# mariohsouto/ProxSDP.jl

Measured on AMD Instinct MI355X. Metric: PDHG iterations/sec at target rank ~ sqrt(n), Max-Cut SDP n=4000 (tol 1e-4 options), higher is better.
Workload: dtype f64

## Files before the change

include/proxsdp_hip.h:

```cpp
#ifndef PROXSDP_HIP_H
#define PROXSDP_HIP_H

#include <stdint.h>

#ifdef __cplusplus
extern "C" {
#endif

#define PROXSDP_HIP_ABI_VERSION 10

#define PROXSDP_E_INVALID  (-1)
#define PROXSDP_E_HIP      (-2)
#define PROXSDP_E_NOMEM    (-3)
#define PROXSDP_E_UNSUPP   (-4)
#define PROXSDP_E_INTERNAL (-5)
#define PROXSDP_E_COMM_ABORTED (-6)

#define PROXSDP_STATUS_NOT_CALLED       0
#define PROXSDP_STATUS_OPTIMAL          1
#define PROXSDP_STATUS_TIME_LIMIT       2
#define PROXSDP_STATUS_ITERATION_LIMIT  3
#define PROXSDP_STATUS_INFEAS_OR_UNBND  4
#define PROXSDP_STATUS_DUAL_INFEASIBLE  5
#define PROXSDP_STATUS_INFEASIBLE       6
// ... 166 lines not shown
    double  host_eig_overlap_time;
    int64_t sign_short_pass;
    int64_t sign_short_fail;
    int64_t full_eigs_lanczos_certified;
    int64_t full_eigs_lanczos_cert_failed;
    int64_t cert_matvecs;
    int64_t dense_truncated_projections;
    int64_t wide_krylov_projections;
    int64_t reserved_s[4];
    int64_t dense_setup_passes;
    int64_t dense_sigma_steps;
} proxsdp_stats;
#define PROXSDP_STATS_SHARDED_GENERAL_ITERATIONS 0
#define PROXSDP_STATS_DEVICE_EIG_MERGES 1
#define PROXSDP_STATS_DEVICE_EIG_MERGE_FALLBACKS 2

typedef struct proxsdp_result {
    int32_t status;
    int32_t certificate_found;
    int32_t primal_feasible_user_tol;
    int32_t dual_feasible_user_tol;
    int32_t result_count;
    int32_t final_rank;
    int64_t iter;
    double  primal_residual;
    double  dual_residual;
    double  objval, dual_objval, gap, time;
    double  dual_feasibility;
    double* primal;
    double* dual_cone;
// ... 260 lines not shown
```

proxsdp.jl_amd/binding.py:

```python
import ctypes as C
import os
import pathlib
import re

import numpy as np
import scipy.sparse as sp

_HERE = pathlib.Path(__file__).resolve().parent
LIB_PATH = _HERE / "libproxsdp_hip.so"
HEADER_PATH = _HERE.parent / "include" / "proxsdp_hip.h"

TRACE_COLS = 14
TRACE_NAMES = ("iter", "prim_obj", "dual_obj", "gap", "feas", "prim_res", "dual_res",
               "primal_step", "beta", "theta", "target_rank", "trials", "elapsed", "matvecs")


class LibraryNotBuilt(RuntimeError):
    pass


class ProxSDPHipError(RuntimeError):
    def __init__(self, code, msg):
        super().__init__(f"libproxsdp_hip error {code}: {msg}")
        self.code = code
# ... 105 lines not shown
                ("dense_truncated_projections", i64), ("wide_krylov_projections", i64), ("reserved_s", i64 * 4),
                ("dense_setup_passes", i64), ("dense_sigma_steps", i64)]


class Result(C.Structure):
    _fields_ = [("status", i32), ("certificate_found", i32), ("primal_feasible_user_tol", i32),
                ("dual_feasible_user_tol", i32), ("result_count", i32), ("final_rank", i32),
                ("iter", i64), ("primal_residual", f64), ("dual_residual", f64),
                ("objval", f64), ("dual_objval", f64), ("gap", f64), ("time", f64),
                ("dual_feasibility", f64),
                ("primal", pf64), ("dual_cone", pf64), ("dual_eq", pf64), ("dual_in", pf64),
                ("slack_eq", pf64), ("slack_in", pf64), ("trace", pf64), ("trace_rows", i64),
                ("status_string", C.c_char * 256), ("stats", Stats)]


STATS_RESERVED_SLOTS = {"sharded_general_iterations": 0, "device_eig_merges": 1, "device_eig_merge_fallbacks": 2}

STATE_NHIST = 7
STATE_HIST_NAMES = ("dual_gap", "prim_obj", "dual_obj", "feasibility", "primal_residual", "dual_residual", "comb_residual")
STATE_SCAL_NAMES = ("primal_step", "primal_step_old", "dual_step", "beta", "theta", "adapt_level",
                    "equa_feasibility", "ineq_feasibility", "dual_feasibility")


class State(C.Structure):
    _fields_ = [("struct_size", i64), ("iteration", i64), ("n", i64), ("Q", i64), ("n_psd", i64), ("hist_len", i64),
                ("x", pf64), ("y", pf64), ("Mty", pf64), ("Mx", pf64),
                ("target_rank", pi64), ("current_rank", pi64), ("min_eig", pf64), ("hist", pf64),
                ("scal", f64 * 16), ("ints", i64 * 8)]


class ShardIO(C.Structure):
# ... 1081 lines not shown
```

proxsdp.jl_amd/csrc/kernels.hip.hpp:

```cpp
#pragma once
#include <hip/hip_runtime.h>
#include <cstdint>

namespace proxsdp {
namespace dev {

constexpr int WAVE = 64;
constexpr int TILE = 64;
constexpr int TPB = 256;
constexpr int NWAVE = TPB / WAVE;
constexpr int CPW = TILE / NWAVE;
constexpr double INV_SQRT2 = 0.70710678118654752440;
constexpr double SQRT2 = 1.41421356237309504880;

#ifdef PX_TIMELINE
constexpr int TL_WG = 160, TL_SLOTS = 8, TL_K = 260;
__device__ unsigned long long g_tl[2][TL_K][TL_WG][TL_SLOTS];
#define PX_TL(kind, k, slot)                                                                                   \
    do {                                                                                                       \
        if (threadIdx.x == 0 && (int)blockIdx.x < ::proxsdp::dev::TL_WG && (k) >= 0 && (k) < ::proxsdp::dev::TL_K) { \
            asm volatile("" ::: "memory");                                                                     \
            ::proxsdp::dev::g_tl[kind][k][blockIdx.x][slot] = wall_clock64();                                    \
            asm volatile("" ::: "memory");                                                                     \
        }                                                                                                      \
// ... 289 lines not shown
    if (wv == 0) wbuf[i] = ((s_acc[0][lane] + s_acc[1][lane]) + (s_acc[2][lane] + s_acc[3][lane])) * INV_SQRT2;
}

__device__ __forceinline__ double fold16_all(double (&t)[16], int lane) {
    fold_stage<8>(t, lane);
    fold_stage<4>(t, lane);
    fold_stage<2>(t, lane);
    fold_stage<1>(t, lane);
    return add_xor32(add_xor16(t[0]));
}
struct FopArgs {
    const double* Vp;
    const double* lam;
    int rp;
    const double* tpart;
    const double* ebuf;
    const double* apart;
};
template <int NCH, int NCHP>
__device__ __forceinline__ void
lz_orth_body(const double* __restrict__ Ppart, int nt, int npad, const double* __restrict__ V, int ldv, int k,
             double* __restrict__ wbuf, const double* __restrict__ hred, double* __restrict__ hpart_out, int pld,
             double* __restrict__ hsum_out, const LanczosCtl* __restrict__ ctl,
             const double* __restrict__ alphas, const double* __restrict__ betas,
             const double* __restrict__ Apart, int napart, int first, const double* __restrict__ arrow, int keep,
             const FopArgs& fo) {
    PX_TL(1, k, 0);
    const int stop = ctl->stop;
    constexpr int NC = 16 * NCH;
    constexpr int NCP = 16 * (NCHP > 0 ? NCHP : 1);
    __shared__ double s_t[NWAVE * 4 * 4 * NCP];
    __shared__ double s_u[4 * NCP];
    __shared__ double s_h[4 * NC];
    __shared__ double s_q[4 * NC];
    __shared__ double s_acc[NWAVE][LZ_ROWS];
    __shared__ double s_red[NWAVE];
    const int lane = threadIdx.x & 63;
    const int wv = __builtin_amdgcn_readfirstlane((int)(threadIdx.x >> 6));
    const int i = blockIdx.x * LZ_ROWS + lane;
    double pv[16];
    double av[8];
    constexpr int NLP = (NCHP > 0 ? NCHP : 1);
    double vrp[NCP], tp[16][NLP], eb = 0.0, ap = 0.0;
    if constexpr (NCHP == 0) {
#pragma unroll
        for (int u = 0; u < 16; ++u) pv[u] = (wv + u * NWAVE < nt) ? Ppart[(long long)(wv + u * NWAVE) * npad + i] : 0.0;
#pragma unroll
        for (int u = 0; u < 8; ++u) av[u] = (u * TPB < napart) ? Apart[min((int)threadIdx.x + u * TPB, napart - 1)] : 0.0;
    } else {
        const int gl0 = min(lane, pld - 1);
#pragma unroll
        for (int c = 0; c < NCP; ++c) {
            const int cc = min(wv + 4 * c, max(fo.rp - 1, 0));
            vrp[c] = fo.Vp[(long long)cc * ldv + i];
        }
#pragma unroll
        for (int u = 0; u < 16; ++u) {
            const long long rec = (long long)min(wv + NWAVE * u, pld - 1) * RLD;
#pragma unroll
            for (int ch = 0; ch < NLP; ++ch)
                tp[u][ch] = ((ch == 0 || 64 * ch < fo.rp) && (wv + NWAVE * u < nt || pld > WAVE)) ? fo.tpart[rec + 64 * ch + lane] : 0.0;
        }
        eb = fo.ebuf[i];
        ap = fo.apart[gl0];
    }
    double vr[NC];
#pragma unroll
    for (int c0 = 0; c0 < NC; c0 += 4) {
        if (wv + 4 * c0 <= k) {
#pragma unroll
            for (int c = c0; c < c0 + 4; ++c) vr[c] = V[(long long)min(wv + 4 * c, k) * ldv + i];
        } else {
#pragma unroll
            for (int c = c0; c < c0 + 4; ++c) vr[c] = 0.0;
        }
    }
// ... 16 lines not shown
    const double binv = first ? 1.0 : 1.0 / be_km;
    if constexpr (NCHP == 0) {
#pragma unroll
        for (int u = 0; u < 16; ++u) if (wv + u * NWAVE >= nt) pv[u] = 0.0;
        double acc = (((pv[0] + pv[1]) + (pv[2] + pv[3])) + ((pv[4] + pv[5]) + (pv[6] + pv[7]))) +
                     (((pv[8] + pv[9]) + (pv[10] + pv[11])) + ((pv[12] + pv[13]) + (pv[14] + pv[15])));
        for (int s = wv + 16 * NWAVE; s < nt; s += NWAVE) acc += Ppart[(long long)s * npad + i];
        s_acc[wv][lane] = acc;
#pragma unroll
        for (int u = 0; u < 8; ++u) if ((int)threadIdx.x + u * TPB >= napart) av[u] = 0.0;
        double a = ((av[0] + av[1]) + (av[2] + av[3])) + ((av[4] + av[5]) + (av[6] + av[7]));
        for (int t = threadIdx.x + 8 * TPB; t < napart; t += TPB) a += Apart[t];
        a = wave_sum(a);
        if (lane == 0) s_red[wv] = a;
    } else {
#pragma unroll
        for (int ch = 0; ch < NLP; ++ch) {
            double pr[16], q4[4];
#pragma unroll
            for (int u = 0; u < 16; ++u) {
                pr[u] = tp[u][ch];
                if (64 * ch < fo.rp)
                    for (int g = wv + NWAVE * u + WAVE; g < pld; g += WAVE) pr[u] += fo.tpart[(long long)g * RLD + 64 * ch + lane];
            }
            tree_in_wave(pr, q4);
#pragma unroll
            for (int a = 0; a < 4; ++a) s_t[(wv * 4 + a) * (64 * NLP) + 64 * ch + lane] = q4[a];
        }
        if (lane >= pld) ap = 0.0;
        else for (int g = lane + WAVE; g < pld; g += WAVE) ap += fo.apart[g];
        ap = wave_sum(ap);
        if (lane == 0) s_red[wv] = (wv == 0) ? ap : 0.0;
    }
    if (!first && (int)threadIdx.x < 4 * NC) s_h[threadIdx.x] = ((int)threadIdx.x < k) ? hred_j : 0.0;
    __syncthreads();
    PX_TL(1, k, 3);
    double alpha, wi;
    if constexpr (NCHP == 0) {
        alpha = ((s_red[0] + s_red[1]) + (s_red[2] + s_red[3])) * INV_SQRT2 * binv * binv;
        wi = ((s_acc[0][lane] + s_acc[1][lane]) + (s_acc[2][lane] + s_acc[3][lane])) * (INV_SQRT2 * binv);
    } else {
        auto tsum = [&](int c) { return tree_across(s_t, 64 * NLP, c); };
        double tl = 0.0;
        if (lane < fo.rp) { const double t0 = tsum(lane); tl = lam_l0 * t0 * t0; }
        if constexpr (NCHP > 1) if (lane + WAVE < fo.rp) { const double t1 = tsum(lane + WAVE); tl += lam_l1 * t1 * t1; }
        tl = wave_sum(tl);
        alpha = (tl + s_red[0]) * binv * binv;
        wi = eb * binv;
        if (j < 4 * NCP) s_u[j] = (j < fo.rp) ? lam_j * tsum(j) : 0.0;
    }
    double ck = alpha;
    if (first) {
        if (j < keep) s_q[j] = f_j;
    } else {
        ck -= s_h[k - 1];
        double fh = 0.0;
        if (keep > 0 && k > keep) {
            if (lane < keep) fh = f_l0 * s_h[lane];
            if (lane + WAVE < keep) fh += f_l1 * s_h[lane + WAVE];
            for (int jj = lane + 2 * WAVE; jj < keep; jj += WAVE) fh += arrow[jj] * s_h[jj];
            fh = wave_sum(fh);
        }
        if (j < k) {
            const double hj = s_h[j];
// ... 42 lines not shown
        const double r = wave_sum(wp * wp);
        if (lane == 0) hpart_out[(long long)pld * KLD + blockIdx.x] = r;
    }
    if (blockIdx.x == 0 && threadIdx.x == 0) hsum_out[k] = ck;
#pragma unroll
    for (int ch = 0; ch < NCH; ++ch) {
        double t[16];
#pragma unroll
        for (int c = 0; c < 16; ++c) t[c] = (wv + 4 * (16 * ch + c) <= k) ? vr[16 * ch + c] * wp : 0.0;
        const double hs = fold16_all(t, lane);
        const int jc = wv + 4 * (16 * ch + lane);
        if (lane < 16 && jc <= k) hpart_out[(long long)blockIdx.x * KLD + jc] = hs;
    }
    PX_TL(1, k, 6);
}
template <int NCH, int NCHP>
__global__ void __launch_bounds__(TPB)
k_lz_orth(const double* __restrict__ Ppart, int nt, int npad, const double* __restrict__ V, int ldv, int k,
          double* __restrict__ wbuf, const double* __restrict__ hred, double* __restrict__ hpart_out, int pld,
          double* __restrict__ hsum_out, const LanczosCtl* __restrict__ ctl,
          const double* __restrict__ alphas, const double* __restrict__ betas,
          const double* __restrict__ Apart, int napart, int first, const double* __restrict__ arrow, int keep,
          FopArgs fo) {
    lz_orth_body<NCH, NCHP>(Ppart, nt, npad, V, ldv, k, wbuf, hred, hpart_out, pld, hsum_out, ctl, alphas, betas, Apart,
                            napart, first, arrow, keep, fo);
}

template <int NCH>
__device__ __forceinline__ void lz_finish_body(const double* __restrict__ wbuf, double* __restrict__ V, int ldv, int k,
                                               const double* __restrict__ hpart_in, int pld,
                                               const double* __restrict__ h1, double* __restrict__ alphas,
                                               double* __restrict__ betas, LanczosCtl* __restrict__ ctl,
                                               double tol, int use_carry, int g,
                                               double* __restrict__ s_h, double* __restrict__ s_d,
                                               double* __restrict__ s_beta, double* __restrict__ hred,
                                               int nprod ) {
    constexpr int NC = 16 * NCH;
    __shared__ double s_p[NWAVE * 4 * 64 * NCH];
    const int lane = threadIdx.x & 63;
    const int wv = __builtin_amdgcn_readfirstlane((int)(threadIdx.x >> 6));
// ... 204 lines not shown
    const LzBlk& b = B.b[blockIdx.z];
    if (b.mode == 0) return;
    FopArgs fo{};
    lz_orth_body<1, 0>(b.Ppart, B.nt, B.npad, b.V, B.npad, b.k, b.wbuf, b.hred, (b.k & 1) ? b.hpart2 : b.hpart1, B.pld,
                       b.hsum, b.ctl, b.alphas, b.betas, b.Apart, B.napart, b.k == b.keep ? 1 : 0, b.arrow, b.keep, fo);
}

struct EllOverflow {
    const int* wr_ptr;
    const int* wr_row;
    const int* wr_lo;
    const int* wr_hi;
    const int* ov_col;
    const int* ov_sidx;
};
template <int NCHP>
__device__ __forceinline__ void fop_body(const double* __restrict__ v, const double* __restrict__ Vp, int ldv, int rp,
                                         const int* __restrict__ ell_col, const int* __restrict__ ell_sidx, int ell_w,
                                         int npad, const double* __restrict__ esv, double* __restrict__ tpart, int pld,
                                         double* __restrict__ ebuf, double* __restrict__ apart, int g,
                                         double* __restrict__ s_e , const LanczosCtl* __restrict__ ctl,
                                         const EllOverflow& ov, int tlk = -1 ) {
    constexpr int NCP = 16 * NCHP;
    const int lane = threadIdx.x & 63;
    const int wv = __builtin_amdgcn_readfirstlane((int)(threadIdx.x >> 6));
    const int i = g * LZ_ROWS + lane;
    PX_TL(0, tlk, 0);
    const int stop = (ctl != nullptr) ? ctl->stop : 0;
    const double vi = v[i];
    double vrp[NCP];
#pragma unroll
    for (int c = 0; c < NCP; ++c) vrp[c] = Vp[(long long)min(wv + 4 * c, max(rp - 1, 0)) * ldv + i];
    int col0[4], sx0[4];
#pragma unroll
    for (int u = 0; u < 4; ++u) {
        const int k = min(wv + u * NWAVE, ell_w - 1);
        col0[u] = ell_col[(long long)k * npad + i];
        sx0[u] = (wv + u * NWAVE < ell_w) ? ell_sidx[(long long)k * npad + i] : -1;
    }
    if (stop) return;
    PX_TL(0, tlk, 1);
    double e = 0.0;
    for (int k0 = wv; k0 < ell_w; k0 += 4 * NWAVE) {
        int col[4], sx[4];
#pragma unroll
        for (int u = 0; u < 4; ++u) {
            if (k0 == wv) { col[u] = col0[u]; sx[u] = sx0[u]; continue; }
// ... 19 lines not shown
                const int rloc = ov.wr_row[q], grow = g * LZ_ROWS + rloc;
                double a = 0.0;
                for (int k = ov.wr_lo[q] + (int)threadIdx.x; k < ov.wr_hi[q]; k += TPB) {
                    const int col = ov.ov_col[k];
                    const double evk = esv[ov.ov_sidx[k]];
                    a += ((col == grow) ? evk : evk * INV_SQRT2) * v[col];
                }
                a = wave_sum(a);
                if (lane == 0) s_w[wv] = a;
                __syncthreads();
                if (threadIdx.x == 0) s_e[rloc] += (s_w[0] + s_w[1]) + (s_w[2] + s_w[3]);
                __syncthreads();
            }
        }
    }
#pragma unroll
    for (int ch = 0; ch < NCHP; ++ch) {
        double t[16];
#pragma unroll
        for (int c = 0; c < 16; ++c) t[c] = vrp[16 * ch + c] * vi;
        const double ts = fold16_all(t, lane);
        const int cc = wv + 4 * (16 * ch + lane);
        if (lane < 16 && cc < rp) tpart[(long long)g * RLD + cc] = ts;
    }
    __syncthreads();
    PX_TL(0, tlk, 3);
    if (wv == 0) {
        const double ei = (s_e[lane] + s_e[LZ_ROWS + lane]) + (s_e[2 * LZ_ROWS + lane] + s_e[3 * LZ_ROWS + lane]);
        ebuf[i] = ei;
        const double a = wave_sum(vi * ei);
        if (lane == 0) apart[g] = a;
    }
    PX_TL(0, tlk, 4);
}
template <int NCHP>
__global__ void __launch_bounds__(TPB)
k_fop(const double* __restrict__ v, const double* __restrict__ Vp, int ldv, int rp,
      const int* __restrict__ ell_col, const int* __restrict__ ell_sidx, int ell_w, int npad,
      const double* __restrict__ esv, double* __restrict__ tpart, int pld, double* __restrict__ ebuf,
      double* __restrict__ apart, const LanczosCtl* __restrict__ ctl, EllOverflow ov) {
    __shared__ double s_e[NWAVE * LZ_ROWS];
    fop_body<NCHP>(v, Vp, ldv, rp, ell_col, ell_sidx, ell_w, npad, esv, tpart, pld, ebuf, apart, blockIdx.x, s_e, ctl, ov);
}
template <int NCHP, int NCH>
__global__ void __launch_bounds__(TPB)
k_fop_finish(const double* __restrict__ wbuf, double* __restrict__ V, int ldv, int k,
             const double* __restrict__ hpart_in, int pld, const double* __restrict__ h1,
             double* __restrict__ alphas, double* __restrict__ betas, LanczosCtl* __restrict__ ctl, double tol,
             int use_carry, int nt, const double* __restrict__ Vp, int rp,
             const int* __restrict__ ell_col, const int* __restrict__ ell_sidx, int ell_w, int npad,
             const double* __restrict__ esv, double* __restrict__ tpart, double* __restrict__ ebuf,
             double* __restrict__ apart, double* __restrict__ hred, EllOverflow ov) {
    __shared__ double s_a[2 * NWAVE * TILE];
    __shared__ double s_b[NWAVE * LZ_ROWS];
    __shared__ double s_beta;
    if ((int)blockIdx.x < nt) {
        lz_finish_body<NCH>(wbuf, V, ldv, k, hpart_in, pld, h1, alphas, betas, ctl, tol, use_carry, blockIdx.x,
                            s_a, s_b, &s_beta, hred, nt);
    } else {
        fop_body<NCHP>(wbuf, Vp, ldv, rp, ell_col, ell_sidx, ell_w, npad, esv, tpart, pld, ebuf, apart,
                       (int)blockIdx.x - nt, s_b, ctl, ov, k + 1);
    }
}

__global__ void __launch_bounds__(TPB)
k_lz_rotate(const double* __restrict__ V, int ldv, int n, int K, const double* __restrict__ U, int ldu,
            int ncols, double* __restrict__ out, int ldo, int copy_src, int copy_dst) {
    extern __shared__ double s_mem[];
    double* s_U = s_mem;
    double* s_V = s_mem + (size_t)K * ncols;
    const int lane = threadIdx.x & 63, wv = threadIdx.x >> 6;
    const int i = blockIdx.x * LZ_ROWS + lane;
    for (int t = threadIdx.x; t < K * ncols; t += TPB) {
        const int j = t % K, c = t / K;
        s_U[t] = U[(long long)c * ldu + j];
    }
// ... 1285 lines not shown
```

proxsdp.jl_amd/csrc/lanczos.hip.hpp:

```cpp
#pragma once
#include "solver.hip.hpp"

namespace proxsdp {

struct LzRecord {
    const double* al; const double* be;
    dev::LanczosCtl ctl;
    LzRecord(const double* rec, int ld) : al(rec), be(rec + ld) { std::memcpy(&ctl, rec + 2 * ld, sizeof(ctl)); }
};

template <typename K, typename... Args>
static inline void launch_prof(EigEvents* prof, K kern, dim3 grid, hipStream_t stream, Args... args) {
    if (!prof) { hipLaunchKernelGGL(kern, grid, dim3(dev::TPB), 0, stream, args...); return; }
    const auto e = prof->acquire();
    hipExtLaunchKernelGGL(kern, grid, dim3(dev::TPB), 0, stream, e.first, e.second, 0, args...);
}
inline EigEvents* Solver::profiled_launch(EigWork& W, int phase) const {
    if (!(opt.profile_symv_every > 0 && (W.lst.symv_launches % opt.profile_symv_every) == phase)) return nullptr;
    return phase == 0 ? &W.ev : &W.evo;
}

inline void Solver::launch_symv(EigWork& W, const double* xp, const double* v, bool use_ctl, dev::LanczosCtl* ctl) {
    EigEvents* const prof = profiled_launch(W, 0);
    if (W.use_fop) {
        auto kern = (W.F_r <= 64) ? dev::k_fop<1> : dev::k_fop<2>;
        launch_prof(prof, kern, dim3(W.nt), stream,
                    v, W.prev_factors().V, W.npad, W.F_r,
                    (const int*)W.ell_col.p, (const int*)W.ell_sidx.p, W.ell_w, W.npad, W.esv, W.tpart.p, W.pld,
                    W.ebuf.p, W.apartf.p, (const dev::LanczosCtl*)(use_ctl ? W.ctl_p : nullptr), W.ov);
    } else {
        launch_prof(prof, dev::k_symv_packed, dim3(W.napart), stream,
                    xp, W.n, W.nt, W.npad, v, W.Ppart.p, (const dev::LanczosCtl*)(use_ctl ? (ctl ? ctl : W.ctl_p) : nullptr), W.Apart.p);
    }
    count_matvecs(W, 1);
}

inline double* lz_hpart(EigWork& W, int k) { return (k & 1) ? W.hpart2.p : W.hpart1.p; }

inline void Solver::launch_symv_finish(EigWork& W, const double* xp, int kclose, double tol, bool use_carry) {
    EigEvents* const prof = profiled_launch(W, 0);
    with_nch(kclose + 1, [&](auto nch) {
        constexpr int NCH = decltype(nch)::value;
        if (W.use_fop) {
            auto kern = (W.F_r <= 64) ? dev::k_fop_finish<1, NCH> : dev::k_fop_finish<2, NCH>;
            launch_prof(prof, kern, dim3(2 * W.nt), stream,
                        (const double*)W.w.p, W.V.p, W.npad, kclose, (const double*)lz_hpart(W, kclose), W.pld,
                        (const double*)W.hsum1.p, W.alphas_p, W.betas_p, W.ctl_p, tol, use_carry ? 1 : 0, W.nt,
                        W.prev_factors().V, W.F_r,
                        (const int*)W.ell_col.p, (const int*)W.ell_sidx.p, W.ell_w, W.npad, W.esv, W.tpart.p, W.ebuf.p,
                        W.apartf.p, W.hred.p, W.ov);
        } else {
            launch_prof(prof, dev::k_symv_finish<NCH>, dim3(W.nt + W.napart), stream,
                        xp, W.n, W.nt, W.npad, W.Ppart.p, (const double*)W.w.p, W.V.p, W.npad, kclose,
                        (const double*)lz_hpart(W, kclose), W.pld, (const double*)W.hsum1.p, W.alphas_p, W.betas_p, W.ctl_p,
                        tol, use_carry ? 1 : 0, W.Apart.p, W.hred.p);
        }
    });
    count_matvecs(W, 1);
}

inline void Solver::lz_launch_finish(EigWork& W, int k, double tol, bool use_carry) {
    with_nch(k + 1, [&](auto nch) {
        hipLaunchKernelGGL(dev::k_lz_finish<decltype(nch)::value>, dim3(W.nt), dim3(dev::TPB), 0, stream,
                           (const double*)W.w.p, W.n, W.V.p, W.npad, k, (const double*)lz_hpart(W, k), W.pld,
                           (const double*)W.hsum1.p, W.alphas_p, W.betas_p, W.ctl_p, tol, use_carry ? 1 : 0, W.hred.p);
    });
}

inline void Solver::lz_launch_begin(EigWork& W, const double* start, dev::LanczosCtl* ctl) {
    hipLaunchKernelGGL(dev::k_lz_begin, dim3(ceil_div(W.npad, dev::TPB)), dim3(dev::TPB), 0, stream,
                       W.V.p, start, W.npad, ctl);
}

inline void Solver::lz_launch_orth(EigWork& W, int k, int first, int keep, EigEvents* prof) {
    dev::FopArgs fo{};
    if (W.use_fop) {
        const EigWork::Factors F = W.prev_factors();
        fo.Vp = F.V; fo.lam = F.lam; fo.rp = F.r;
        fo.tpart = W.tpart.p; fo.ebuf = W.ebuf.p; fo.apart = W.apartf.p;
    }
    auto launch_orth = [&](auto kern) {
        launch_prof(prof, kern, dim3(W.nt), stream,
                    (const double*)W.Ppart.p, W.nt, W.npad, (const double*)W.V.p, W.npad, k, W.w.p,
                    (const double*)W.hred.p, lz_hpart(W, k), W.pld, W.hsum1.p,
                    (const dev::LanczosCtl*)W.ctl_p, (const double*)W.alphas_p, (const double*)W.betas_p,
                    (const double*)W.Apart.p, W.napart, first, (const double*)W.arrow_p, keep, fo);
    };
    with_nch(k + 1, [&](auto nch) {
        constexpr int NCH = decltype(nch)::value;
        if (!W.use_fop) launch_orth(dev::k_lz_orth<NCH, 0>);
        else if (W.F_r <= 64) launch_orth(dev::k_lz_orth<NCH, 1>);
        else launch_orth(dev::k_lz_orth<NCH, 2>);
    });
}

inline void Solver::lz_first_matvec(EigWork& W, const double* xp, int k, bool& presymv, dev::LanczosCtl* ctl) {
    if (!presymv) launch_symv(W, xp, W.V.p + (size_t)k * W.npad, true, ctl);
    else count_matvecs(W, 1);
    presymv = false;
}

inline void Solver::lz_launch_step(EigWork& W, const double* xp, int k, int kfirst, double step_tol, bool& presymv) {
    if (k == kfirst) lz_first_matvec(W, xp, k, presymv, W.ctl_p);
    else launch_symv_finish(W, xp, k - 1, step_tol, k - 1 > kfirst);
    lz_launch_orth(W, k, k == kfirst ? 1 : 0, kfirst, profiled_launch(W, 1));
}

// ... 187 lines not shown
    return true;
}

inline void Solver::lz_plan(EigWork& W, LzRun& R, bool single_block) {
    LzPlan& p = R.plan;
    const int krylovdim = R.krylovdim;
    const bool wide = krylovdim > dev::LZ_KMAX;
    const int merge_from = opt.host_eig_merge == 0 ? (1 << 30) : (opt.host_eig_merge == 1 ? 24 : 64);
    const bool split_wanted = single_block && !R.arpack && krylovdim >= merge_from;
    const bool blk1 = single_block && !wide && block1_plan(W, krylovdim, split_wanted);
    p.engine = wide ? LzEngine::wide : blk1 ? LzEngine::block1 : LzEngine::step;
    p.rec = W.record(wide);
    p.split = p.engine == LzEngine::step && split_wanted;
    p.dev_wanted = p.split && (opt.device_eig_merge == 1 || (opt.device_eig_merge < 0 && krylovdim >= 64));
    p.dev_merge = p.dev_wanted && rot_sink == nullptr && StreamRef::tl == nullptr && DeviceMerge::eligible(krylovdim);
}

inline void Solver::lz_prepare_arrow(LzRun& R) {
    R.m_arrow = R.kfirst;
    if (R.m_arrow <= 0) return;
    const int n1 = R.m_arrow + 1, ld = R.ld;
    R.Qa.assign((size_t)n1 * n1, 0.0); R.da.assign(n1, 0.0); R.ea.assign(n1, 0.0);
    for (int j = 0; j < R.m_arrow; ++j) {
        R.Qa[(size_t)j * n1 + j] = R.T[(size_t)j * ld + j];
        R.Qa[(size_t)j * n1 + R.m_arrow] = R.Qa[(size_t)R.m_arrow * n1 + j] = R.T[(size_t)j * ld + R.m_arrow];
    }
    householder_tridiag(n1, R.Qa.data(), R.da.data(), R.ea.data());
}

inline bool Solver::lz_split_first(EigWork& W, LzRun& R) {
// ... 562 lines not shown
```

proxsdp.jl_amd/csrc/pdhg_loop.hip.hpp:

```cpp
#pragma once
#include "solver.hip.hpp"

namespace proxsdp {

constexpr int PSTRIDE = 2048;
constexpr int NQ = 16;

inline void Solver::spmv(const double* x, double* y) {
    spmv_sparse(x, y);
    if (P.dense()) dense_mv(x, y, true);
}
inline void Solver::spmv_sparse(const double* x, double* y) {
    if (P.Q == 0) return;
    if (csr_wave)
        hipLaunchKernelGGL(dev::k_spmv_csr_wave, dim3(ceil_div(P.Q, dev::NWAVE)), dim3(dev::TPB), 0, stream,
                           csr_ptr.p, csr_col.p, csr_val.p, x, y, (int)P.Q, LONG_ROW);
    else
        hipLaunchKernelGGL(dev::k_spmv_csr_thread, dim3(ceil_div(P.Q, dev::TPB)), dim3(dev::TPB), 0, stream,
                           csr_ptr.p, csr_col.p, csr_val.p, x, y, (int)P.Q, LONG_ROW);
    if (n_seg > 0) {
        hipLaunchKernelGGL(dev::k_spmv_csr_seg, dim3(n_seg), dim3(dev::TPB), 0, stream,
                           seg_lo_d.p, seg_hi_d.p, csr_col.p, csr_val.p, x, segpart_d.p);
        hipLaunchKernelGGL(dev::k_spmv_seg_fin, dim3(ceil_div(n_long, dev::TPB)), dim3(dev::TPB), 0, stream,
                           long_row_d.p, long_ptr_d.p, n_long, segpart_d.p, y);
// ... 820 lines not shown
                        whi.push_back((int)ocol.size());
                    }
                    wptr[g + 1] = (int)wrow.size();
                }
                W.wr_ptr.alloc(wptr.size()); W.wr_row.alloc(wrow.size()); W.wr_lo.alloc(wlo.size()); W.wr_hi.alloc(whi.size());
                W.ov_col.alloc(ocol.size()); W.ov_sidx.alloc(osx.size());
                W.wr_ptr.upload(wptr.data(), wptr.size(), stream); W.wr_row.upload(wrow.data(), wrow.size(), stream);
                W.wr_lo.upload(wlo.data(), wlo.size(), stream); W.wr_hi.upload(whi.data(), whi.size(), stream);
                W.ov_col.upload(ocol.data(), ocol.size(), stream); W.ov_sidx.upload(osx.data(), osx.size(), stream);
                W.ov = dev::EllOverflow{W.wr_ptr.p, W.wr_row.p, W.wr_lo.p, W.wr_hi.p, W.ov_col.p, W.ov_sidx.p};
                PX_HIP(hipStreamSynchronize(stream));
            }
            W.F.alloc((size_t)W.npad * W.cap); W.F.zero(stream);
            W.Flam.alloc(std::max(W.n, dev::MAXK)); W.Flam.zero(stream);
            W.tpart.alloc((size_t)dev::MAXK * W.pld); W.tpart.zero(stream);
            W.ebuf.alloc(W.npad); W.ebuf.zero(stream);
            W.apartf.alloc(W.pld); W.apartf.zero(stream);
            W.warm_part.alloc(ceil_div(W.npad, dev::TPB)); W.warm_part.zero(stream);
            PX_HIP(hipStreamSynchronize(stream));
            W.fop_ok = true;
        }
    }
    PX_HIP(hipStreamSynchronize(stream));
    use_support = true;
}

inline void Solver::upload_sparse_operator() {
    std::vector<int> rp(P.Q + 1), cp(P.n + 1);
    for (int64_t i = 0; i <= P.Q; ++i) rp[i] = (int)P.rowptr[i];
    for (int64_t i = 0; i <= P.n; ++i) cp[i] = (int)P.colptr[i];
// ... 689 lines not shown
```

proxsdp.jl_amd/csrc/solver.hip.hpp:

```cpp
#pragma once
#include <hip/hip_runtime.h>
#include <hip/hip_ext.h>
#include <array>
#include <memory>
#include <mutex>
#include <condition_variable>
#include <functional>
#include <exception>
#include <rocblas/rocblas.h>
#include <rocsolver/rocsolver.h>

#include <algorithm>
#include <chrono>
#include <cmath>
#include <cstdio>
#include <cstdlib>
#include <cstring>
#include <stdexcept>
#include <string>
#include <thread>
#include <tuple>
#include <type_traits>
#include <utility>
#include <vector>
// ... 172 lines not shown

struct StreamRef {
    Stream main;
    static inline thread_local hipStream_t tl = nullptr;
    operator hipStream_t() const { return tl ? tl : main.h; }
};

struct LzRecBuf { double* dev = nullptr; double* host = nullptr; size_t doubles = 0; int ld = 0; dev::LanczosCtl* ctl = nullptr; };
enum class LzEngine { step, block1, wide };
struct LzPlan {
    LzEngine engine = LzEngine::step;
    LzRecBuf rec;
    bool split = false;
    bool dev_wanted = false;
    bool dev_merge = false;
};
struct LzRun {
    LzPlan plan;
    int nev = 0, krylovdim = 0, ld = 0;
    bool arpack = false, positive_part = false;
    double tol = 0.0, step_tol = 0.0;
    long long maxiter = 0;
    std::vector<double> T, Tw, D, U, f, al, be, Qa, da, ea;
    int howmany = 0, numiter = 1, converged = 0, K = 0, kfirst = 0, pos_count = -1, m_arrow = 0;
    bool pos_fail = false, presymv = false;
    double betaK = 0.0;
    int k1 = 0;
    bool split_cycle = false, split_ready = false;
    bool merge_active = false;
    bool dev_staged = false;
// ... 23 lines not shown
    dev::LanczosCtl* ctlw_p = nullptr;
    static constexpr size_t RECW_DOUBLES = 2 * dev::LZW_MAXK + sizeof(dev::LanczosCtl) / sizeof(double);
    LzRecBuf record(bool wide_one) const {
        if (wide_one) return {recw.p, recw_pinned.p, RECW_DOUBLES, dev::LZW_MAXK, ctlw_p};
        return {rec.p, rec_host, REC_DOUBLES, dev::MAXK, ctl_p};
    }
    DevBuf<double> A, D, E;
    DevBuf<rocblas_int> info;
    std::vector<double> resid_host;
    PinnedBuf Ustage[2];
    int ustage_next = 0;
    int rot_form = 0, rot_launches = 0;
    std::vector<double> vals;
    int count = 0, converged_eigs = 0, numiter = 0, prev_numiter = 1;
    bool converged = false;
    DevBuf<double> F, Flam, tpart, ebuf, apartf;
    DevBuf<int> ell_col, ell_sidx;
    DevBuf<int> wr_ptr, wr_row, wr_lo, wr_hi, ov_col, ov_sidx;
    dev::EllOverflow ov{};
    int ell_w = 0, F_first = 0, F_r = 0;
    bool fop_ok = false;
    bool have_factors = false;
    bool use_fop = false;
    struct XPrev {
        bool sparse = true;
        int last_npos = -1;
    } xprev;
    struct Factors { const double* V; const double* lam; int r; };
    Factors prev_factors() const { return {F.p + (size_t)F_first * npad, Flam.p, F_r}; }
    void forget_factors() { have_factors = false; xprev.sparse = false; use_fop = false; }
    bool ritz_ok = false;
// ... 129 lines not shown
    struct BatchCtx {
        DevBuf<double> U;
        PinnedBuf U_host, rec_host;
        std::unique_ptr<SpinPool> pool;
        Event ev;
    };
    std::vector<std::unique_ptr<BatchCtx>> batch_ctx;
    std::mutex batch_stats_mu;
    std::unique_ptr<SpinPool> merge_pool;
    ParFor merge_par;
    int merge_helpers() const { return opt.host_merge_threads < 0 ? 3 : std::min(15, (int)opt.host_merge_threads); }
    static constexpr size_t LZB_USTRIDE = 64 * 64 + 2 * dev::MAXK;
    int block1_lds_cap = 0;
    DevBuf<long long> b1_dbg;
    bool sg48_ok = false;
    EigEvents* profiled_launch(EigWork& W, int phase) const;
    void launch_symv(EigWork& W, const double* xp, const double* v, bool use_ctl, dev::LanczosCtl* ctl = nullptr);
    void launch_symv_finish(EigWork& W, const double* xp, int kclose, double tol, bool use_carry);
    void lz_launch_finish(EigWork& W, int k, double tol, bool use_carry);
    void lz_launch_begin(EigWork& W, const double* start, dev::LanczosCtl* ctl);
    void lz_launch_orth(EigWork& W, int k, int first, int keep, EigEvents* prof);
    void lz_first_matvec(EigWork& W, const double* xp, int k, bool& presymv, dev::LanczosCtl* ctl);
    void lz_launch_step(EigWork& W, const double* xp, int k, int kfirst, double step_tol, bool& presymv);
    void lzw_step(EigWork& W, LzRun& R, const double* xp, int k);
    bool block1_plan(const EigWork& W, int krylovdim, bool split_wanted) const;
    void launch_block1(EigWork& W, const double* xp, int kfirst, int krylovdim, double tol);
    void lz_read_record(const LzRecBuf& rec, double* dst, hipStream_t s);
    void rotate(EigWork& W, int K, const std::vector<double>& U, int ldu, int ncols, double* out, int copy_src, int copy_dst,
                const double* extra, int nextra);
    void rotate_launch(EigWork& W, int K, const double* Ud, int ncols, double* out, int copy_src, int copy_dst);
// ... 332 lines not shown
    sg48_ok = true;
    for (const void* f : {reinterpret_cast<const void*>(dev::k_sym_gemm48<dev::SG_PLAIN, 4>), reinterpret_cast<const void*>(dev::k_sym_gemm48<dev::SG_POLY, 4>)})
        sg48_ok = sg48_ok && hipFuncSetAttribute(f, hipFuncAttributeMaxDynamicSharedMemorySize, (int)dev::sg48_lds_bytes(4)) == hipSuccess;
    if (!sg48_ok) (void)hipGetLastError();
    small_sign_cap = 0;
    for (int sd : {64, 56, 48, 40, 32, 24, 16}) {
        const size_t bytes = dev::small_sign_lds_bytes(sd);
        if (bytes <= 48 * 1024 || hipFuncSetAttribute(reinterpret_cast<const void*>(dev::k_small_sign_project),
                                                      hipFuncAttributeMaxDynamicSharedMemorySize, (int)bytes) == hipSuccess) {
            small_sign_cap = sd;
            break;
        }
        (void)hipGetLastError();
    }
    if (std::getenv("PROXSDP_HIP_DEBUG_B1") != nullptr) { b1_dbg.alloc(8); b1_dbg.zero(stream); }
    block1_lds_cap = 0;
    for (int kb : {160, 144, 128, 112, 96}) {
        bool ok = true;
        for (const void* f : {reinterpret_cast<const void*>(dev::k_lz_block1<1, false>), reinterpret_cast<const void*>(dev::k_lz_block1<2, false>),
                              reinterpret_cast<const void*>(dev::k_lz_block1<1, true>), reinterpret_cast<const void*>(dev::k_lz_block1<2, true>)})
            ok = ok && hipFuncSetAttribute(f, hipFuncAttributeMaxDynamicSharedMemorySize, kb * 1024) == hipSuccess;
        if (ok) { block1_lds_cap = kb * 1024; break; }
        (void)hipGetLastError();
    }
    blas.create();
    PX_ROC(rocblas_set_stream(blas, stream));
}

inline void Solver::start_rocsolver_warmup() {
    const int dev_id = opt.device_id;
// ... 294 lines not shown
        PX_MERGE(lanczos_matvecs); PX_MERGE(lanczos_restarts); PX_MERGE(lanczos_calls);
        PX_MERGE(full_eigs); PX_MERGE(krylov_fallbacks);
        PX_MERGE(symv_launches); PX_MERGE(symv_bytes);
        PX_MERGE(symv_profiled); PX_MERGE(symv_profiled_ms);
        PX_MERGE(orth_profiled); PX_MERGE(orth_profiled_ms);
        PX_MERGE(full_eig_solver_ms); PX_MERGE(full_eig_recon_ms);
        PX_MERGE(full_eigs_lanczos); PX_MERGE(full_eigs_lanczos_checks); PX_MERGE(full_eigs_lanczos_mismatches);
        PX_MERGE(full_eigs_lanczos_certified); PX_MERGE(full_eigs_lanczos_cert_failed); PX_MERGE(cert_matvecs);
        PX_MERGE(dense_truncated_projections); PX_MERGE(wide_krylov_projections);
        PX_MERGE(full_eigs_sign); PX_MERGE(sign_products); PX_MERGE(sign_short_pass); PX_MERGE(sign_short_fail);
        PX_MERGE(sign_engine_projections); PX_MERGE(sign_engine_rejected);
        PX_MERGE(sign_engine_checks); PX_MERGE(sign_engine_mismatches);
        PX_MERGE(batched_block_steps);
        PX_MERGE(host_eigs); PX_MERGE(host_eig_time); PX_MERGE(host_eig_merges); PX_MERGE(host_eig_overlap_time);
        PX_MERGE(reserved_s[PROXSDP_STATS_DEVICE_EIG_MERGES]); PX_MERGE(reserved_s[PROXSDP_STATS_DEVICE_EIG_MERGE_FALLBACKS]);
        PX_MERGE(warm_starts); PX_MERGE(device_eigs); PX_MERGE(mfma_reconstructions);
        PX_MERGE(cycle_launches); PX_MERGE(cycle_steps); PX_MERGE(cycle_ms);
        PX_MERGE(fop_projections);
        a = proxsdp_stats{};
        lz_matvec_iter += W.mv_iter; recon_r_iter += W.recon_r;
        W.mv_iter = 0; W.recon_r = 0;
    }
#undef PX_MERGE
}

}
```

Baseline: 556.8.

## Add owner workgroups computing full projection dot products in fused Lanczos matvec

Adds extra 'owner' workgroups to the fused low-rank-plus-sparse matvec kernels. Each owner computes one or two full dot products of the Lanczos vector with previous factor columns and writes the reduced result to a small buffer. The orthogonalization kernel then reads those reduced values directly instead of loading and tree-reducing per-tile partials across all tiles, and the main tiles skip writing their partials. The cost is more workgroups per launch, each doing a long serial read over the whole vector, which could lengthen the critical path if the owners finish later than the sparse tiles. It is enabled by default for single-block step-engine runs and can be turned off with an environment variable.

New measurement: 610.3 (median of 6 runs). 1.1x the previous value.

```diff
diff --git a/include/proxsdp_hip.h b/include/proxsdp_hip.h
--- a/include/proxsdp_hip.h
+++ b/include/proxsdp_hip.h
@@ -204,6 +204,7 @@
 #define PROXSDP_STATS_SHARDED_GENERAL_ITERATIONS 0
 #define PROXSDP_STATS_DEVICE_EIG_MERGES 1
 #define PROXSDP_STATS_DEVICE_EIG_MERGE_FALLBACKS 2
+#define PROXSDP_STATS_FOP_OWNER_STEPS 3
 
 typedef struct proxsdp_result {
     int32_t status;
diff --git a/proxsdp.jl_amd/binding.py b/proxsdp.jl_amd/binding.py
--- a/proxsdp.jl_amd/binding.py
+++ b/proxsdp.jl_amd/binding.py
@@ -143,7 +143,8 @@
                 ("status_string", C.c_char * 256), ("stats", Stats)]
 
 
-STATS_RESERVED_SLOTS = {"sharded_general_iterations": 0, "device_eig_merges": 1, "device_eig_merge_fallbacks": 2}
+STATS_RESERVED_SLOTS = {"sharded_general_iterations": 0, "device_eig_merges": 1, "device_eig_merge_fallbacks": 2,
+                        "fop_owner_steps": 3}
 
 STATE_NHIST = 7
 STATE_HIST_NAMES = ("dual_gap", "prim_obj", "dual_obj", "feasibility", "primal_residual", "dual_residual", "comb_residual")
diff --git a/proxsdp.jl_amd/csrc/kernels.hip.hpp b/proxsdp.jl_amd/csrc/kernels.hip.hpp
--- a/proxsdp.jl_amd/csrc/kernels.hip.hpp
+++ b/proxsdp.jl_amd/csrc/kernels.hip.hpp
@@ -327,10 +327,11 @@
     const double* lam;
     int rp;
     const double* tpart;
+    const double* tred;
     const double* ebuf;
     const double* apart;
 };
-template <int NCH, int NCHP>
+template <int NCH, int NCHP, bool OWN = false>
 __device__ __forceinline__ void
 lz_orth_body(const double* __restrict__ Ppart, int nt, int npad, const double* __restrict__ V, int ldv, int k,
              double* __restrict__ wbuf, const double* __restrict__ hred, double* __restrict__ hpart_out, int pld,
@@ -342,7 +343,7 @@
     const int stop = ctl->stop;
     constexpr int NC = 16 * NCH;
     constexpr int NCP = 16 * (NCHP > 0 ? NCHP : 1);
-    __shared__ double s_t[NWAVE * 4 * 4 * NCP];
+    __shared__ double s_t[OWN ? 1 : NWAVE * 4 * 4 * NCP];
     __shared__ double s_u[4 * NCP];
     __shared__ double s_h[4 * NC];
     __shared__ double s_q[4 * NC];
@@ -354,7 +355,8 @@
     double pv[16];
     double av[8];
     constexpr int NLP = (NCHP > 0 ? NCHP : 1);
-    double vrp[NCP], tp[16][NLP], eb = 0.0, ap = 0.0;
+    double vrp[NCP], tp[OWN ? 1 : 16][NLP], eb = 0.0, ap = 0.0;
+    double t_j = 0.0, t_l0 = 0.0, t_l1 = 0.0;
     if constexpr (NCHP == 0) {
 #pragma unroll
         for (int u = 0; u < 16; ++u) pv[u] = (wv + u * NWAVE < nt) ? Ppart[(long long)(wv + u * NWAVE) * npad + i] : 0.0;
@@ -367,12 +369,18 @@
             const int cc = min(wv + 4 * c, max(fo.rp - 1, 0));
             vrp[c] = fo.Vp[(long long)cc * ldv + i];
         }
-#pragma unroll
-        for (int u = 0; u < 16; ++u) {
-            const long long rec = (long long)min(wv + NWAVE * u, pld - 1) * RLD;
-#pragma unroll
-            for (int ch = 0; ch < NLP; ++ch)
-                tp[u][ch] = ((ch == 0 || 64 * ch < fo.rp) && (wv + NWAVE * u < nt || pld > WAVE)) ? fo.tpart[rec + 64 * ch + lane] : 0.0;
+        if constexpr (OWN) {
+            t_j = fo.tred[min((int)threadIdx.x, RLD - 1)];
+            t_l0 = fo.tred[lane];
+            if constexpr (NCHP > 1) t_l1 = fo.tred[lane + WAVE];
+        } else {
+#pragma unroll
+            for (int u = 0; u < 16; ++u) {
+                const long long rec = (long long)min(wv + NWAVE * u, pld - 1) * RLD;
+#pragma unroll
+                for (int ch = 0; ch < NLP; ++ch)
+                    tp[u][ch] = ((ch == 0 || 64 * ch < fo.rp) && (wv + NWAVE * u < nt || pld > WAVE)) ? fo.tpart[rec + 64 * ch + lane] : 0.0;
+            }
         }
         eb = fo.ebuf[i];
         ap = fo.apart[gl0];
@@ -419,18 +427,20 @@
         a = wave_sum(a);
         if (lane == 0) s_red[wv] = a;
     } else {
-#pragma unroll
-        for (int ch = 0; ch < NLP; ++ch) {
-            double pr[16], q4[4];
-#pragma unroll
-            for (int u = 0; u < 16; ++u) {
-                pr[u] = tp[u][ch];
-                if (64 * ch < fo.rp)
-                    for (int g = wv + NWAVE * u + WAVE; g < pld; g += WAVE) pr[u] += fo.tpart[(long long)g * RLD + 64 * ch + lane];
+        if constexpr (!OWN) {
+#pragma unroll
+            for (int ch = 0; ch < NLP; ++ch) {
+                double pr[16], q4[4];
+#pragma unroll
+                for (int u = 0; u < 16; ++u) {
+                    pr[u] = tp[u][ch];
+                    if (64 * ch < fo.rp)
+                        for (int g = wv + NWAVE * u + WAVE; g < pld; g += WAVE) pr[u] += fo.tpart[(long long)g * RLD + 64 * ch + lane];
+                }
+                tree_in_wave(pr, q4);
+#pragma unroll
+                for (int a = 0; a < 4; ++a) s_t[(wv * 4 + a) * (64 * NLP) + 64 * ch + lane] = q4[a];
             }
-            tree_in_wave(pr, q4);
-#pragma unroll
-            for (int a = 0; a < 4; ++a) s_t[(wv * 4 + a) * (64 * NLP) + 64 * ch + lane] = q4[a];
         }
         if (lane >= pld) ap = 0.0;
         else for (int g = lane + WAVE; g < pld; g += WAVE) ap += fo.apart[g];
@@ -445,14 +455,17 @@
         alpha = ((s_red[0] + s_red[1]) + (s_red[2] + s_red[3])) * INV_SQRT2 * binv * binv;
         wi = ((s_acc[0][lane] + s_acc[1][lane]) + (s_acc[2][lane] + s_acc[3][lane])) * (INV_SQRT2 * binv);
     } else {
-        auto tsum = [&](int c) { return tree_across(s_t, 64 * NLP, c); };
+        auto tsum = [&](int c, double own) {
+            if constexpr (OWN) return own;
+            else return tree_across(s_t, 64 * NLP, c);
+        };
         double tl = 0.0;
-        if (lane < fo.rp) { const double t0 = tsum(lane); tl = lam_l0 * t0 * t0; }
-        if constexpr (NCHP > 1) if (lane + WAVE < fo.rp) { const double t1 = tsum(lane + WAVE); tl += lam_l1 * t1 * t1; }
+        if (lane < fo.rp) { const double t0 = tsum(lane, t_l0); tl = lam_l0 * t0 * t0; }
+        if constexpr (NCHP > 1) if (lane + WAVE < fo.rp) { const double t1 = tsum(lane + WAVE, t_l1); tl += lam_l1 * t1 * t1; }
         tl = wave_sum(tl);
         alpha = (tl + s_red[0]) * binv * binv;
         wi = eb * binv;
-        if (j < 4 * NCP) s_u[j] = (j < fo.rp) ? lam_j * tsum(j) : 0.0;
+        if (j < 4 * NCP) s_u[j] = (j < fo.rp) ? lam_j * tsum(j, t_j) : 0.0;
     }
     double ck = alpha;
     if (first) {
@@ -525,7 +538,7 @@
     }
     PX_TL(1, k, 6);
 }
-template <int NCH, int NCHP>
+template <int NCH, int NCHP, bool OWN = false>
 __global__ void __launch_bounds__(TPB)
 k_lz_orth(const double* __restrict__ Ppart, int nt, int npad, const double* __restrict__ V, int ldv, int k,
           double* __restrict__ wbuf, const double* __restrict__ hred, double* __restrict__ hpart_out, int pld,
@@ -533,8 +546,8 @@
           const double* __restrict__ alphas, const double* __restrict__ betas,
           const double* __restrict__ Apart, int napart, int first, const double* __restrict__ arrow, int keep,
           FopArgs fo) {
-    lz_orth_body<NCH, NCHP>(Ppart, nt, npad, V, ldv, k, wbuf, hred, hpart_out, pld, hsum_out, ctl, alphas, betas, Apart,
-                            napart, first, arrow, keep, fo);
+    lz_orth_body<NCH, NCHP, OWN>(Ppart, nt, npad, V, ldv, k, wbuf, hred, hpart_out, pld, hsum_out, ctl, alphas, betas, Apart,
+                                 napart, first, arrow, keep, fo);
 }
 
 template <int NCH>
@@ -769,7 +782,46 @@
     const int* ov_col;
     const int* ov_sidx;
 };
-template <int NCHP>
+__device__ __forceinline__ void fop_owner_body(const double* __restrict__ v, const double* __restrict__ Vp, int ldv, int rp,
+                                               int nt, double* __restrict__ tred, int g, const LanczosCtl* __restrict__ ctl) {
+    __shared__ double s_o[2 * NWAVE * 4];
+    const int lane = threadIdx.x & 63;
+    const int wv = __builtin_amdgcn_readfirstlane((int)(threadIdx.x >> 6));
+    const bool own1 = g + nt < rp;
+    if (g >= rp) return;
+    const int stop = (ctl != nullptr) ? ctl->stop : 0;
+    double vb[16], vc0[16], vc1[16];
+#pragma unroll
+    for (int u = 0; u < 16; ++u) {
+        const long long r = (long long)min(wv + NWAVE * u, nt - 1) * LZ_ROWS + lane;
+        vb[u] = v[r];
+        vc0[u] = Vp[(long long)g * ldv + r];
+        if (own1) vc1[u] = Vp[(long long)(g + nt) * ldv + r];
+    }
+    if (stop) return;
+    auto own_col = [&](const double (&vc)[16], int slot) {
+        double t[16];
+#pragma unroll
+        for (int u = 0; u < 16; ++u) t[u] = (wv + NWAVE * u < nt) ? vc[u] * vb[u] : 0.0;
+        double s = fold16_all(t, lane);
+        s = s + lane_xor<2>(s);
+        s = s + lane_xor<1>(s);
+        if (lane < 16 && (lane & 3) == 0) s_o[(slot * NWAVE + wv) * 4 + (lane >> 2)] = s;
+    };
+    own_col(vc0, 0);
+    if (own1) own_col(vc1, 1);
+    __syncthreads();
+    if (wv == 0) {
+        const int q = lane & 3, sl = (lane >> 2) & 1;
+        const double* so = s_o + sl * NWAVE * 4 + q;
+        double a = (so[0 * 4] + so[2 * 4]) + (so[1 * 4] + so[3 * 4]);
+        a = a + lane_xor<1>(a);
+        a = a + lane_xor<2>(a);
+        if (lane == 0) tred[g] = a;
+        if (lane == 4 && own1) tred[g + nt] = a;
+    }
+}
+template <int NCHP, bool REC = true>
 __device__ __forceinline__ void fop_body(const double* __restrict__ v, const double* __restrict__ Vp, int ldv, int rp,
                                          const int* __restrict__ ell_col, const int* __restrict__ ell_sidx, int ell_w,
                                          int npad, const double* __restrict__ esv, double* __restrict__ tpart, int pld,
@@ -783,9 +835,11 @@
     PX_TL(0, tlk, 0);
     const int stop = (ctl != nullptr) ? ctl->stop : 0;
     const double vi = v[i];
-    double vrp[NCP];
-#pragma unroll
-    for (int c = 0; c < NCP; ++c) vrp[c] = Vp[(long long)min(wv + 4 * c, max(rp - 1, 0)) * ldv + i];
+    [[maybe_unused]] double vrp[REC ? NCP : 1];
+    if constexpr (REC) {
+#pragma unroll
+        for (int c = 0; c < NCP; ++c) vrp[c] = Vp[(long long)min(wv + 4 * c, max(rp - 1, 0)) * ldv + i];
+    }
     int col0[4], sx0[4];
 #pragma unroll
     for (int u = 0; u < 4; ++u) {
@@ -835,14 +889,16 @@
             }
         }
     }
-#pragma unroll
-    for (int ch = 0; ch < NCHP; ++ch) {
-        double t[16];
-#pragma unroll
-        for (int c = 0; c < 16; ++c) t[c] = vrp[16 * ch + c] * vi;
-        const double ts = fold16_all(t, lane);
-        const int cc = wv + 4 * (16 * ch + lane);
-        if (lane < 16 && cc < rp) tpart[(long long)g * RLD + cc] = ts;
+    if constexpr (REC) {
+#pragma unroll
+        for (int ch = 0; ch < NCHP; ++ch) {
+            double t[16];
+#pragma unroll
+            for (int c = 0; c < 16; ++c) t[c] = vrp[16 * ch + c] * vi;
+            const double ts = fold16_all(t, lane);
+            const int cc = wv + 4 * (16 * ch + lane);
+            if (lane < 16 && cc < rp) tpart[(long long)g * RLD + cc] = ts;
+        }
     }
     __syncthreads();
     PX_TL(0, tlk, 3);
@@ -854,16 +910,20 @@
     }
     PX_TL(0, tlk, 4);
 }
-template <int NCHP>
+template <int NCHP, bool OWN = false>
 __global__ void __launch_bounds__(TPB)
 k_fop(const double* __restrict__ v, const double* __restrict__ Vp, int ldv, int rp,
       const int* __restrict__ ell_col, const int* __restrict__ ell_sidx, int ell_w, int npad,
       const double* __restrict__ esv, double* __restrict__ tpart, int pld, double* __restrict__ ebuf,
-      double* __restrict__ apart, const LanczosCtl* __restrict__ ctl, EllOverflow ov) {
+      double* __restrict__ apart, const LanczosCtl* __restrict__ ctl, EllOverflow ov, double* __restrict__ tred) {
     __shared__ double s_e[NWAVE * LZ_ROWS];
-    fop_body<NCHP>(v, Vp, ldv, rp, ell_col, ell_sidx, ell_w, npad, esv, tpart, pld, ebuf, apart, blockIdx.x, s_e, ctl, ov);
-}
-template <int NCHP, int NCH>
+    if constexpr (OWN) {
+        const int nt = (int)gridDim.x / 2;
+        if ((int)blockIdx.x >= nt) { fop_owner_body(v, Vp, ldv, rp, nt, tred, (int)blockIdx.x - nt, ctl); return; }
+    }
+    fop_body<NCHP, !OWN>(v, Vp, ldv, rp, ell_col, ell_sidx, ell_w, npad, esv, tpart, pld, ebuf, apart, blockIdx.x, s_e, ctl, ov);
+}
+template <int NCHP, int NCH, bool OWN = false>
 __global__ void __launch_bounds__(TPB)
 k_fop_finish(const double* __restrict__ wbuf, double* __restrict__ V, int ldv, int k,
              const double* __restrict__ hpart_in, int pld, const double* __restrict__ h1,
@@ -871,7 +931,7 @@
              int use_carry, int nt, const double* __restrict__ Vp, int rp,
              const int* __restrict__ ell_col, const int* __restrict__ ell_sidx, int ell_w, int npad,
              const double* __restrict__ esv, double* __restrict__ tpart, double* __restrict__ ebuf,
-             double* __restrict__ apart, double* __restrict__ hred, EllOverflow ov) {
+             double* __restrict__ apart, double* __restrict__ hred, EllOverflow ov, double* __restrict__ tred) {
     __shared__ double s_a[2 * NWAVE * TILE];
     __shared__ double s_b[NWAVE * LZ_ROWS];
     __shared__ double s_beta;
@@ -879,8 +939,11 @@
         lz_finish_body<NCH>(wbuf, V, ldv, k, hpart_in, pld, h1, alphas, betas, ctl, tol, use_carry, blockIdx.x,
                             s_a, s_b, &s_beta, hred, nt);
     } else {
-        fop_body<NCHP>(wbuf, Vp, ldv, rp, ell_col, ell_sidx, ell_w, npad, esv, tpart, pld, ebuf, apart,
-                       (int)blockIdx.x - nt, s_b, ctl, ov, k + 1);
+        if constexpr (OWN) {
+            if ((int)blockIdx.x >= 2 * nt) { fop_owner_body(wbuf, Vp, ldv, rp, nt, tred, (int)blockIdx.x - 2 * nt, ctl); return; }
+        }
+        fop_body<NCHP, !OWN>(wbuf, Vp, ldv, rp, ell_col, ell_sidx, ell_w, npad, esv, tpart, pld, ebuf, apart,
+                             (int)blockIdx.x - nt, s_b, ctl, ov, k + 1);
     }
 }
 
diff --git a/proxsdp.jl_amd/csrc/lanczos.hip.hpp b/proxsdp.jl_amd/csrc/lanczos.hip.hpp
--- a/proxsdp.jl_amd/csrc/lanczos.hip.hpp
+++ b/proxsdp.jl_amd/csrc/lanczos.hip.hpp
@@ -20,14 +20,20 @@
     return phase == 0 ? &W.ev : &W.evo;
 }
 
+inline bool lz_fop_owner(const EigWork& W) {
+    return W.use_fop && W.lzrun.plan.fop_owner && W.pld <= dev::WAVE && W.F_r > 0 && W.F_r <= 2 * W.nt;
+}
+
 inline void Solver::launch_symv(EigWork& W, const double* xp, const double* v, bool use_ctl, dev::LanczosCtl* ctl) {
     EigEvents* const prof = profiled_launch(W, 0);
     if (W.use_fop) {
-        auto kern = (W.F_r <= 64) ? dev::k_fop<1> : dev::k_fop<2>;
-        launch_prof(prof, kern, dim3(W.nt), stream,
+        const bool own = lz_fop_owner(W);
+        auto kern = own ? ((W.F_r <= 64) ? dev::k_fop<1, true> : dev::k_fop<2, true>)
+                        : ((W.F_r <= 64) ? dev::k_fop<1> : dev::k_fop<2>);
+        launch_prof(prof, kern, dim3(own ? 2 * W.nt : W.nt), stream,
                     v, W.prev_factors().V, W.npad, W.F_r,
                     (const int*)W.ell_col.p, (const int*)W.ell_sidx.p, W.ell_w, W.npad, W.esv, W.tpart.p, W.pld,
-                    W.ebuf.p, W.apartf.p, (const dev::LanczosCtl*)(use_ctl ? W.ctl_p : nullptr), W.ov);
+                    W.ebuf.p, W.apartf.p, (const dev::LanczosCtl*)(use_ctl ? W.ctl_p : nullptr), W.ov, W.tred.p);
     } else {
         launch_prof(prof, dev::k_symv_packed, dim3(W.napart), stream,
                     xp, W.n, W.nt, W.npad, v, W.Ppart.p, (const dev::LanczosCtl*)(use_ctl ? (ctl ? ctl : W.ctl_p) : nullptr), W.Apart.p);
@@ -42,13 +48,15 @@
     with_nch(kclose + 1, [&](auto nch) {
         constexpr int NCH = decltype(nch)::value;
         if (W.use_fop) {
-            auto kern = (W.F_r <= 64) ? dev::k_fop_finish<1, NCH> : dev::k_fop_finish<2, NCH>;
-            launch_prof(prof, kern, dim3(2 * W.nt), stream,
+            const bool own = lz_fop_owner(W);
+            auto kern = own ? ((W.F_r <= 64) ? dev::k_fop_finish<1, NCH, true> : dev::k_fop_finish<2, NCH, true>)
+                            : ((W.F_r <= 64) ? dev::k_fop_finish<1, NCH> : dev::k_fop_finish<2, NCH>);
+            launch_prof(prof, kern, dim3((own ? 3 : 2) * W.nt), stream,
                         (const double*)W.w.p, W.V.p, W.npad, kclose, (const double*)lz_hpart(W, kclose), W.pld,
                         (const double*)W.hsum1.p, W.alphas_p, W.betas_p, W.ctl_p, tol, use_carry ? 1 : 0, W.nt,
                         W.prev_factors().V, W.F_r,
-                        (const int*)W.ell_col.p, (const int*)W.ell_sidx.p, W.ell_w, W.npad, W.esv, W.tpart.p, W.ebuf.p,
-                        W.apartf.p, W.hred.p, W.ov);
+                        (const int*)W.ell_col.p, (const int*)W.ell_sidx.p, W.ell_w, W.npad, W.esv, W.tpart.p,
+                        W.ebuf.p, W.apartf.p, W.hred.p, W.ov, W.tred.p);
         } else {
             launch_prof(prof, dev::k_symv_finish<NCH>, dim3(W.nt + W.napart), stream,
                         xp, W.n, W.nt, W.npad, W.Ppart.p, (const double*)W.w.p, W.V.p, W.npad, kclose,
@@ -77,8 +85,10 @@
     if (W.use_fop) {
         const EigWork::Factors F = W.prev_factors();
         fo.Vp = F.V; fo.lam = F.lam; fo.rp = F.r;
-        fo.tpart = W.tpart.p; fo.ebuf = W.ebuf.p; fo.apart = W.apartf.p;
-    }
+        fo.tpart = W.tpart.p; fo.tred = W.tred.p; fo.ebuf = W.ebuf.p; fo.apart = W.apartf.p;
+    }
+    const bool own = lz_fop_owner(W);
+    if (own) W.lst.reserved_s[PROXSDP_STATS_FOP_OWNER_STEPS]++;
     auto launch_orth = [&](auto kern) {
         launch_prof(prof, kern, dim3(W.nt), stream,
                     (const double*)W.Ppart.p, W.nt, W.npad, (const double*)W.V.p, W.npad, k, W.w.p,
@@ -89,8 +99,8 @@
     with_nch(k + 1, [&](auto nch) {
         constexpr int NCH = decltype(nch)::value;
         if (!W.use_fop) launch_orth(dev::k_lz_orth<NCH, 0>);
-        else if (W.F_r <= 64) launch_orth(dev::k_lz_orth<NCH, 1>);
-        else launch_orth(dev::k_lz_orth<NCH, 2>);
+        else if (W.F_r <= 64) { if (own) launch_orth(dev::k_lz_orth<NCH, 1, true>); else launch_orth(dev::k_lz_orth<NCH, 1>); }
+        else { if (own) launch_orth(dev::k_lz_orth<NCH, 2, true>); else launch_orth(dev::k_lz_orth<NCH, 2>); }
     });
 }
 
@@ -308,6 +318,8 @@
     p.split = p.engine == LzEngine::step && split_wanted;
     p.dev_wanted = p.split && (opt.device_eig_merge == 1 || (opt.device_eig_merge < 0 && krylovdim >= 64));
     p.dev_merge = p.dev_wanted && rot_sink == nullptr && StreamRef::tl == nullptr && DeviceMerge::eligible(krylovdim);
+    p.fop_owner = single_block && fop_owner_knob != 0 && W.use_fop && p.engine == LzEngine::step && W.tred.n > 0 &&
+                  W.pld <= dev::WAVE && W.F_r > 0 && W.F_r <= 2 * W.nt;
 }
 
 inline void Solver::lz_prepare_arrow(LzRun& R) {
diff --git a/proxsdp.jl_amd/csrc/pdhg_loop.hip.hpp b/proxsdp.jl_amd/csrc/pdhg_loop.hip.hpp
--- a/proxsdp.jl_amd/csrc/pdhg_loop.hip.hpp
+++ b/proxsdp.jl_amd/csrc/pdhg_loop.hip.hpp
@@ -858,6 +858,7 @@
             W.F.alloc((size_t)W.npad * W.cap); W.F.zero(stream);
             W.Flam.alloc(std::max(W.n, dev::MAXK)); W.Flam.zero(stream);
             W.tpart.alloc((size_t)dev::MAXK * W.pld); W.tpart.zero(stream);
+            W.tred.alloc(dev::RLD); W.tred.zero(stream);
             W.ebuf.alloc(W.npad); W.ebuf.zero(stream);
             W.apartf.alloc(W.pld); W.apartf.zero(stream);
             W.warm_part.alloc(ceil_div(W.npad, dev::TPB)); W.warm_part.zero(stream);
diff --git a/proxsdp.jl_amd/csrc/solver.hip.hpp b/proxsdp.jl_amd/csrc/solver.hip.hpp
--- a/proxsdp.jl_amd/csrc/solver.hip.hpp
+++ b/proxsdp.jl_amd/csrc/solver.hip.hpp
@@ -210,6 +210,7 @@
     bool split = false;
     bool dev_wanted = false;
     bool dev_merge = false;
+    bool fop_owner = false;
 };
 struct LzRun {
     LzPlan plan;
@@ -263,7 +264,7 @@
     std::vector<double> vals;
     int count = 0, converged_eigs = 0, numiter = 0, prev_numiter = 1;
     bool converged = false;
-    DevBuf<double> F, Flam, tpart, ebuf, apartf;
+    DevBuf<double> F, Flam, tpart, tred, ebuf, apartf;
     DevBuf<int> ell_col, ell_sidx;
     DevBuf<int> wr_ptr, wr_row, wr_lo, wr_hi, ov_col, ov_sidx;
     dev::EllOverflow ov{};
@@ -423,6 +424,7 @@
     int block1_lds_cap = 0;
     DevBuf<long long> b1_dbg;
     bool sg48_ok = false;
+    int fop_owner_knob = -1;
     EigEvents* profiled_launch(EigWork& W, int phase) const;
     void launch_symv(EigWork& W, const double* xp, const double* v, bool use_ctl, dev::LanczosCtl* ctl = nullptr);
     void launch_symv_finish(EigWork& W, const double* xp, int kclose, double tol, bool use_carry);
@@ -785,6 +787,7 @@
         (void)hipGetLastError();
     }
     if (std::getenv("PROXSDP_HIP_DEBUG_B1") != nullptr) { b1_dbg.alloc(8); b1_dbg.zero(stream); }
+    if (const char* env = std::getenv("PROXSDP_HIP_FOP_OWNER")) fop_owner_knob = (env[0] == '0' && env[1] == 0) ? 0 : -1;
     block1_lds_cap = 0;
     for (int kb : {160, 144, 128, 112, 96}) {
         bool ok = true;
@@ -1109,6 +1112,7 @@
         PX_MERGE(batched_block_steps);
         PX_MERGE(host_eigs); PX_MERGE(host_eig_time); PX_MERGE(host_eig_merges); PX_MERGE(host_eig_overlap_time);
         PX_MERGE(reserved_s[PROXSDP_STATS_DEVICE_EIG_MERGES]); PX_MERGE(reserved_s[PROXSDP_STATS_DEVICE_EIG_MERGE_FALLBACKS]);
+        PX_MERGE(reserved_s[PROXSDP_STATS_FOP_OWNER_STEPS]);
         PX_MERGE(warm_starts); PX_MERGE(device_eigs); PX_MERGE(mfma_reconstructions);
         PX_MERGE(cycle_launches); PX_MERGE(cycle_steps); PX_MERGE(cycle_ms);
         PX_MERGE(fop_projections);
```
